# fabiocarrara/neural-ode-features

Measured on AMD Instinct MI355X. Metric: images/sec (fwd+adjoint) CIFAR-10 ODE-ResNet bs=128 at 1/2/4/8 GPU, higher is better.
Workload: dtype f32

## Files before the change

neural-ode-features_amd/csrc/kernels_head.hip:

```cpp
#include "node_internal.h"
#include "../../include/node_hip.h"
#include <cstdio>

namespace node {

namespace {
constexpr int HEAD_MAXIT = 16;

template <int CTRL>
__device__ inline float dpp_add(float v) {
  return v + __builtin_bit_cast(float, __builtin_amdgcn_update_dpp(0, __builtin_bit_cast(int, v), CTRL, 0xf, 0xf, true));
}
template <int LPC>
__device__ inline float lanes_sum(float v) {
  if (LPC >= 4) { v = dpp_add<0xB1>(v); v = dpp_add<0x4E>(v); }
  if (LPC >= 16) { v = dpp_add<0x141>(v); v = dpp_add<0x140>(v); }
  if (LPC >= 64) {
    v = v + __builtin_bit_cast(float, __builtin_amdgcn_update_dpp(0, __builtin_bit_cast(int, v), 0x142, 0xa, 0xf, false));
    v = v + __builtin_bit_cast(float, __builtin_amdgcn_update_dpp(0, __builtin_bit_cast(int, v), 0x143, 0xc, 0xf, false));
    v = __builtin_bit_cast(float, __builtin_amdgcn_readlane(__builtin_bit_cast(int, v), 63));
  }
  return v;
}

__device__ inline void groups_from_channels(const float* chv, float* grp, int G, int cpg) {
  __syncthreads();
  for (int g = threadIdx.x; g < G; g += blockDim.x) {
    float s = 0.f;
    for (int k = 0; k < cpg; ++k) s += chv[g * cpg + k];
    grp[g] = s;
  }
  __syncthreads();
}

__device__ inline float block_sum_256h(float v, float* red) {
  v = lanes_sum<64>(v);
  __syncthreads();
  if ((threadIdx.x & 63) == 0) red[threadIdx.x >> 6] = v;
  __syncthreads();
  return (red[0] + red[1]) + (red[2] + red[3]);
}

__device__ inline float group_sum(float v, float* ch, int c, int c_lo, int cpg, bool on) {
  __syncthreads();
  if (on) ch[c] = v;
  __syncthreads();
  float s = 0.f;
  if (on)
    for (int k = 0; k < cpg; ++k) s += ch[c_lo + k];
  return s;
}
}

template <int LPC>
__global__ __launch_bounds__(256) void k_head_fwd_v(const float* __restrict__ z, const float* __restrict__ gamma,
                                                    const float* __restrict__ beta, const float* __restrict__ scale,
                                                    float* __restrict__ pooled, float* __restrict__ stats, int C, int HW,
                                                    int G, float eps) {
  extern __shared__ float sm[];
  float* chv = sm;
  float* grp = sm + C;
  float* grp2 = grp + G;
  constexpr int CPP = 256 / LPC;
  const int n = blockIdx.x, cpg = C / G;
  const int lc = threadIdx.x / LPC, lq = threadIdx.x % LPC;
  const int q4 = HW >> 2;
  const int iters = (C + CPP - 1) / CPP;
  const float4* zs = reinterpret_cast<const float4*>(z + (size_t)n * C * HW);
  float4 v[HEAD_MAXIT];
#pragma unroll
  for (int i = 0; i < HEAD_MAXIT; ++i) {
    const int c = i * CPP + lc;
    v[i] = (i < iters && c < C) ? zs[(size_t)c * q4 + lq] : make_float4(0.f, 0.f, 0.f, 0.f);
  }
  const float inv_m = 1.0f / (float)(cpg * HW);
#pragma unroll
  for (int i = 0; i < HEAD_MAXIT; ++i) {
    const int c = i * CPP + lc;
    const float s = lanes_sum<LPC>((v[i].x + v[i].y) + (v[i].z + v[i].w));
    if (i < iters && c < C && lq == 0) chv[c] = s;
  }
  groups_from_channels(chv, grp, G, cpg);
#pragma unroll
  for (int i = 0; i < HEAD_MAXIT; ++i) {
    const int c = i * CPP + lc;
    const float mean = (i < iters && c < C) ? grp[c / cpg] * inv_m : 0.f;
    const float a = v[i].x - mean, b = v[i].y - mean, cc = v[i].z - mean, dd = v[i].w - mean;
    const float s = lanes_sum<LPC>((a * a + b * b) + (cc * cc + dd * dd));
    if (i < iters && c < C && lq == 0) chv[c] = s;
  }
  groups_from_channels(chv, grp2, G, cpg);
#pragma unroll
  for (int i = 0; i < HEAD_MAXIT; ++i) {
    const int c = i * CPP + lc;
    if (i < iters && c < C) {
      const int g = c / cpg;
      const float mean = grp[g] * inv_m, rstd = 1.0f / sqrtf(grp2[g] * inv_m + eps);
      const float gm = gamma[c], bt = beta[c];
      float acc = fmaxf(((v[i].x - mean) * rstd) * gm + bt, 0.f) + fmaxf(((v[i].y - mean) * rstd) * gm + bt, 0.f) +
                  fmaxf(((v[i].z - mean) * rstd) * gm + bt, 0.f) + fmaxf(((v[i].w - mean) * rstd) * gm + bt, 0.f);
      acc = lanes_sum<LPC>(acc) * (1.0f / (float)HW);
      if (lq == 0) {
        if (scale) acc *= scale[(size_t)n * C + c];
        pooled[(size_t)n * C + c] = acc;
        if (c == g * cpg) { stats[((size_t)n * G + g) * 2] = mean; stats[((size_t)n * G + g) * 2 + 1] = rstd; }
      }
    } else {
      (void)lanes_sum<LPC>(0.f);
    }
  }
}

template <int LPC>
__global__ __launch_bounds__(256) void k_head_bwd_v(const float* __restrict__ z, const float* __restrict__ gamma,
                                                    const float* __restrict__ beta, const float* __restrict__ scale,
                                                    const float* __restrict__ stats, const float* __restrict__ gpool,
                                                    float* __restrict__ dz, float* __restrict__ gpart, int C, int HW, int G) {
  extern __shared__ float sm[];
  float* chv = sm;
  float* chw = sm + C;
  float* grp = chw + C;
  float* grp2 = grp + G;
  constexpr int CPP = 256 / LPC;
  const int n = blockIdx.x, cpg = C / G;
  const int lc = threadIdx.x / LPC, lq = threadIdx.x % LPC;
  const int q4 = HW >> 2;
  const int iters = (C + CPP - 1) / CPP;
  const float4* zs = reinterpret_cast<const float4*>(z + (size_t)n * C * HW);
  float4* dzs = reinterpret_cast<float4*>(dz + (size_t)n * C * HW);
  const float inv_m = 1.0f / (float)(cpg * HW);
  float4 xh[HEAD_MAXIT];
  float gvv[HEAD_MAXIT];
#pragma unroll
  for (int i = 0; i < HEAD_MAXIT; ++i) {
    const int c = i * CPP + lc;
    const bool on = i < iters && c < C;
    float4 zv = on ? zs[(size_t)c * q4 + lq] : make_float4(0.f, 0.f, 0.f, 0.f);
    const int g = on ? c / cpg : 0;
    const float mean = on ? stats[((size_t)n * G + g) * 2] : 0.f, rstd = on ? stats[((size_t)n * G + g) * 2 + 1] : 0.f;
    xh[i] = make_float4((zv.x - mean) * rstd, (zv.y - mean) * rstd, (zv.z - mean) * rstd, (zv.w - mean) * rstd);
    float gv = 0.f;
    if (on) {
      gv = gpool[(size_t)n * C + c] * (1.0f / (float)HW);
      if (scale) gv *= scale[(size_t)n * C + c];
    }
    gvv[i] = gv;
    const float gm = on ? gamma[c] : 0.f, bt = on ? beta[c] : 0.f;
    const float g0 = (xh[i].x * gm + bt > 0.f) ? gv : 0.f, g1 = (xh[i].y * gm + bt > 0.f) ? gv : 0.f;
    const float g2 = (xh[i].z * gm + bt > 0.f) ? gv : 0.f, g3 = (xh[i].w * gm + bt > 0.f) ? gv : 0.f;
    const float dg = lanes_sum<LPC>((g0 * xh[i].x + g1 * xh[i].y) + (g2 * xh[i].z + g3 * xh[i].w));
    const float db = lanes_sum<LPC>((g0 + g1) + (g2 + g3));
    if (on && lq == 0) {
      gpart[((size_t)n * 2 + 0) * C + c] = dg;
      gpart[((size_t)n * 2 + 1) * C + c] = db;
      chv[c] = db * gm;
      chw[c] = dg * gm;
    }
  }
  __syncthreads();
  for (int g = threadIdx.x; g < G; g += 256) {
    float s1 = 0.f, s2 = 0.f;
    for (int k = 0; k < cpg; ++k) { s1 += chv[g * cpg + k]; s2 += chw[g * cpg + k]; }
    grp[g] = s1 * inv_m;
    grp2[g] = s2 * inv_m;
  }
  __syncthreads();
#pragma unroll
  for (int i = 0; i < HEAD_MAXIT; ++i) {
    const int c = i * CPP + lc;
    if (i < iters && c < C) {
      const int g = c / cpg;
      const float rstd = stats[((size_t)n * G + g) * 2 + 1], m1 = grp[g], m2 = grp2[g];
      const float gm = gamma[c], bt = beta[c], gv = gvv[i];
      float4 o;
      o.x = rstd * (((xh[i].x * gm + bt > 0.f) ? gv * gm : 0.f) - m1 - xh[i].x * m2);
      o.y = rstd * (((xh[i].y * gm + bt > 0.f) ? gv * gm : 0.f) - m1 - xh[i].y * m2);
      o.z = rstd * (((xh[i].z * gm + bt > 0.f) ? gv * gm : 0.f) - m1 - xh[i].z * m2);
      o.w = rstd * (((xh[i].w * gm + bt > 0.f) ? gv * gm : 0.f) - m1 - xh[i].w * m2);
      dzs[(size_t)c * q4 + lq] = o;
    }
  }
}

__global__ __launch_bounds__(256) void k_head_fwd_g(const float* __restrict__ z, const float* __restrict__ gamma,
                                                    const float* __restrict__ beta, const float* __restrict__ scale,
                                                    float* __restrict__ pooled, float* __restrict__ stats, int C, int HW,
                                                    int G, float eps) {
  extern __shared__ float ch[];
  const int n = blockIdx.x, cpg = C / G;
  const float inv_m = 1.0f / (float)(cpg * HW);
  for (int cb = 0; cb < C; cb += 256) {
    const int c = cb + threadIdx.x;
    const bool on = c < C;
    const int g = on ? c / cpg : 0, c_lo = g * cpg;
    const float* zc = z + ((size_t)n * C + (on ? c : 0)) * HW;
    float s = 0.f;
    if (on)
      for (int p = 0; p < HW; ++p) s += zc[p];
    const float mean = group_sum(s, ch, c, c_lo, cpg, on) * inv_m;
    float s2 = 0.f;
    if (on)
      for (int p = 0; p < HW; ++p) { const float dv = zc[p] - mean; s2 += dv * dv; }
    const float var = group_sum(s2, ch, c, c_lo, cpg, on) * inv_m;
    const float rstd = 1.0f / sqrtf(var + eps);
    if (on) {
      const float gm = gamma[c], bt = beta[c];
      float acc = 0.f;
      for (int p = 0; p < HW; ++p) acc += fmaxf(((zc[p] - mean) * rstd) * gm + bt, 0.f);
      acc *= 1.0f / (float)HW;
      if (scale) acc *= scale[(size_t)n * C + c];
      pooled[(size_t)n * C + c] = acc;
      if (c == c_lo) { stats[((size_t)n * G + g) * 2] = mean; stats[((size_t)n * G + g) * 2 + 1] = rstd; }
    }
  }
}

__global__ __launch_bounds__(256) void k_head_bwd_g(const float* __restrict__ z, const float* __restrict__ gamma,
                                                    const float* __restrict__ beta, const float* __restrict__ scale,
                                                    const float* __restrict__ stats, const float* __restrict__ gpool,
                                                    float* __restrict__ dz, float* __restrict__ gpart, int C, int HW, int G) {
  extern __shared__ float ch[];
  const int n = blockIdx.x, cpg = C / G;
  const float inv_m = 1.0f / (float)(cpg * HW);
  for (int cb = 0; cb < C; cb += 256) {
    const int c = cb + threadIdx.x;
    const bool on = c < C;
    const int g = on ? c / cpg : 0, c_lo = g * cpg;
    const size_t base = ((size_t)n * C + (on ? c : 0)) * HW;
    const float mean = on ? stats[((size_t)n * G + g) * 2] : 0.f, rstd = on ? stats[((size_t)n * G + g) * 2 + 1] : 0.f;
    const float gm = on ? gamma[c] : 0.f, bt = on ? beta[c] : 0.f;
    float gv = 0.f;
    if (on) {
      gv = gpool[(size_t)n * C + c] * (1.0f / (float)HW);
      if (scale) gv *= scale[(size_t)n * C + c];
    }
    float dg = 0.f, db = 0.f;
    if (on)
      for (int p = 0; p < HW; ++p) {
        const float xh = (z[base + p] - mean) * rstd;
        const float gu = (xh * gm + bt > 0.f) ? gv : 0.f;
        dg += gu * xh;
        db += gu;
      }
    if (on) {
      gpart[((size_t)n * 2 + 0) * C + c] = dg;
      gpart[((size_t)n * 2 + 1) * C + c] = db;
    }
    const float m1 = group_sum(db * gm, ch, c, c_lo, cpg, on) * inv_m;
    const float m2 = group_sum(dg * gm, ch, c, c_lo, cpg, on) * inv_m;
    if (on)
      for (int p = 0; p < HW; ++p) {
        const float xh = (z[base + p] - mean) * rstd;
        const float gu = (xh * gm + bt > 0.f) ? gv : 0.f;
        dz[base + p] = rstd * (gu * gm - m1 - xh * m2);
      }
  }
}

__global__ __launch_bounds__(256) void k_gn_relu_fwd(const float* __restrict__ z, const float* __restrict__ gamma,
                                                     const float* __restrict__ beta, float* __restrict__ out,
                                                     float* __restrict__ stats, int C, int HW, int G, float eps, int relu) {
  __shared__ float red[4];
  const int n = blockIdx.x / G, g = blockIdx.x - n * G, cpg = C / G;
  const int M = cpg * HW;
  const size_t base = ((size_t)n * C + (size_t)g * cpg) * HW;
  const float* zg = z + base;
  float s = 0.f;
  for (int i = threadIdx.x; i < M; i += 256) s += zg[i];
  const float mean = block_sum_256h(s, red) / (float)M;
  float s2 = 0.f;
  for (int i = threadIdx.x; i < M; i += 256) { const float dv = zg[i] - mean; s2 += dv * dv; }
  const float rstd = 1.0f / sqrtf(block_sum_256h(s2, red) / (float)M + eps);
  if (threadIdx.x == 0) { stats[(size_t)blockIdx.x * 2] = mean; stats[(size_t)blockIdx.x * 2 + 1] = rstd; }
  for (int cc = 0; cc < cpg; ++cc) {
    const float gm = gamma[g * cpg + cc], bt = beta[g * cpg + cc];
    for (int p = threadIdx.x; p < HW; p += 256) {
      float v = ((zg[cc * HW + p] - mean) * rstd) * gm + bt;
      if (relu) v = fmaxf(v, 0.f);
      out[base + cc * HW + p] = v;
    }
  }
}

__global__ __launch_bounds__(256) void k_gn_relu_bwd(const float* __restrict__ z, const float* __restrict__ gamma,
                                                     const float* __restrict__ beta, const float* __restrict__ stats,
                                                     const float* __restrict__ gout, float* __restrict__ dz,
                                                     float* __restrict__ gpart, int C, int HW, int G, int relu) {
  __shared__ float red[4];
  const int n = blockIdx.x / G, g = blockIdx.x - n * G, cpg = C / G;
  const int M = cpg * HW;
  const size_t base = ((size_t)n * C + (size_t)g * cpg) * HW;
  const float mean = stats[(size_t)blockIdx.x * 2], rstd = stats[(size_t)blockIdx.x * 2 + 1];
  float s1 = 0.f, s2 = 0.f;
  for (int cc = 0; cc < cpg; ++cc) {
    const int c = g * cpg + cc;
    const float gm = gamma[c], bt = beta[c];
    float dg = 0.f, db = 0.f;
    for (int p = threadIdx.x; p < HW; p += 256) {
      const float xh = (z[base + cc * HW + p] - mean) * rstd;
      float gu = gout[base + cc * HW + p];
      if (relu && !(xh * gm + bt > 0.f)) gu = 0.f;
      dg += gu * xh;
      db += gu;
    }
    dg = block_sum_256h(dg, red);
    db = block_sum_256h(db, red);
    if (threadIdx.x == 0) {
      gpart[((size_t)n * 2 + 0) * C + c] = dg;
      gpart[((size_t)n * 2 + 1) * C + c] = db;
    }
    s1 += db * gm;
    s2 += dg * gm;
  }
  const float m1 = s1 / (float)M, m2 = s2 / (float)M;
  for (int cc = 0; cc < cpg; ++cc) {
    const float gm = gamma[g * cpg + cc], bt = beta[g * cpg + cc];
    for (int p = threadIdx.x; p < HW; p += 256) {
      const float xh = (z[base + cc * HW + p] - mean) * rstd;
      float gu = gout[base + cc * HW + p];
      if (relu && !(xh * gm + bt > 0.f)) gu = 0.f;
      dz[base + cc * HW + p] = rstd * (gu * gm - m1 - xh * m2);
    }
  }
}

void launch_gn_relu_fwd(const node_shape& sh, const float* z, const float* gamma, const float* beta, int relu, float* out,
                        float* stats, hipStream_t s) {
  hipLaunchKernelGGL(k_gn_relu_fwd, dim3(sh.n * sh.groups), dim3(256), 0, s, z, gamma, beta, out, stats, sh.c, sh.h * sh.w,
                     sh.groups, sh.eps, relu);
}
void launch_gn_relu_bwd(const node_shape& sh, const float* z, const float* gamma, const float* beta, const float* stats,
                        int relu, const float* gout, float* dz, float* gpart, hipStream_t s) {
  hipLaunchKernelGGL(k_gn_relu_bwd, dim3(sh.n * sh.groups), dim3(256), 0, s, z, gamma, beta, stats, gout, dz, gpart, sh.c,
                     sh.h * sh.w, sh.groups, relu);
}

int head_check(const node_shape* sh, char* why, size_t why_len) {
  if (!sh) { snprintf(why, why_len, "shape is NULL"); return NODE_ERR_NULL; }
  if (sh->n <= 0 || sh->c <= 0 || sh->h <= 0 || sh->w <= 0 || sh->groups <= 0) { snprintf(why, why_len, "non-positive dimension"); return NODE_ERR_SHAPE; }
  if (sh->c % sh->groups != 0) { snprintf(why, why_len, "groups (%d) must divide channels (%d)", sh->groups, sh->c); return NODE_ERR_SHAPE; }
  const int cpg = sh->c / sh->groups;
  if (sh->c > 256 && 256 % cpg != 0) { snprintf(why, why_len, "C = %d with %d channels per group: groups would straddle the 256-channel passes", sh->c, cpg); return NODE_ERR_UNSUPPORTED; }
  if ((size_t)sh->c * sizeof(float) > 24 * 1024) { snprintf(why, why_len, "C = %d does not fit the LDS scratch", sh->c); return NODE_ERR_UNSUPPORTED; }
  return NODE_OK;
}

static int head_lpc(const node_shape& sh) {
  const int HW = sh.h * sh.w;
  if (HW % 4 != 0) return 0;
  const int q4 = HW / 4;
  if (q4 != 1 && q4 != 4 && q4 != 16 && q4 != 64) return 0;
  const int cpp = 256 / q4;
  if ((sh.c + cpp - 1) / cpp > HEAD_MAXIT) return 0;
  return q4;
}

void launch_head_fwd(const node_shape& sh, const float* z, const float* gamma, const float* beta, const float* scale,
                     float* pooled, float* stats, hipStream_t s) {
  const int HW = sh.h * sh.w;
  const size_t lds = (size_t)(sh.c + 2 * sh.groups) * sizeof(float);
#define HEAD_FWD(LPC) hipLaunchKernelGGL((k_head_fwd_v<LPC>), dim3(sh.n), dim3(256), lds, s, z, gamma, beta, scale, pooled, stats, sh.c, HW, sh.groups, sh.eps)
  switch (head_lpc(sh)) {
    case 1: HEAD_FWD(1); return;
    case 4: HEAD_FWD(4); return;
    case 16: HEAD_FWD(16); return;
    case 64: HEAD_FWD(64); return;
    default: break;
  }
#undef HEAD_FWD
  hipLaunchKernelGGL(k_head_fwd_g, dim3(sh.n), dim3(256), (size_t)sh.c * sizeof(float), s, z, gamma, beta, scale, pooled, stats,
                     sh.c, HW, sh.groups, sh.eps);
}
__global__ __launch_bounds__(256) void k_head_gsum(const float* __restrict__ gpart, float* __restrict__ gsum, int N, int W) {
  __shared__ float red[4][64];
  const int col = blockIdx.x * 64 + (threadIdx.x & 63), part = threadIdx.x >> 6;
  float s = 0.f;
  if (col < W)
    for (int n = part; n < N; n += 4) s += gpart[(size_t)n * W + col];
  red[part][threadIdx.x & 63] = s;
  __syncthreads();
  if (part == 0 && col < W) gsum[col] = (red[0][threadIdx.x] + red[1][threadIdx.x]) + (red[2][threadIdx.x] + red[3][threadIdx.x]);
}
void launch_head_gsum(const float* gpart, float* gsum, int N, int C, hipStream_t s) {
  hipLaunchKernelGGL(k_head_gsum, dim3((2 * C + 63) / 64), dim3(256), 0, s, gpart, gsum, N, 2 * C);
}

void launch_head_bwd(const node_shape& sh, const float* z, const float* gamma, const float* beta, const float* scale,
                     const float* stats, const float* gpool, float* dz, float* gpart, hipStream_t s) {
  const int HW = sh.h * sh.w;
  const size_t lds = (size_t)(2 * sh.c + 2 * sh.groups) * sizeof(float);
#define HEAD_BWD(LPC) hipLaunchKernelGGL((k_head_bwd_v<LPC>), dim3(sh.n), dim3(256), lds, s, z, gamma, beta, scale, stats, gpool, dz, gpart, sh.c, HW, sh.groups)
  switch (head_lpc(sh)) {
    case 1: HEAD_BWD(1); return;
    case 4: HEAD_BWD(4); return;
    case 16: HEAD_BWD(16); return;
    case 64: HEAD_BWD(64); return;
    default: break;
  }
#undef HEAD_BWD
  hipLaunchKernelGGL(k_head_bwd_g, dim3(sh.n), dim3(256), (size_t)sh.c * sizeof(float), s, z, gamma, beta, scale, stats, gpool, dz,
                     gpart, sh.c, HW, sh.groups);
}

}
```

neural-ode-features_amd/csrc/kernels_optim.hip:

```cpp
#include "node_internal.h"

namespace node {

__global__ __launch_bounds__(256) void k_sgd_multi(SgdTable tb, float lr, float momentum, float wd, float gscale, const float* skip) {
  if (skip != nullptr && *skip != 0.f) return;
  const SgdEntry e = tb.e[blockIdx.y];
  float* __restrict__ p = e.p;
  const float* __restrict__ g = e.g;
  float* __restrict__ m = e.m;
  const size_t n = e.n;
  const size_t stride = (size_t)gridDim.x * 256;
  const size_t start = (size_t)blockIdx.x * 256 + threadIdx.x;
  const bool vec = (((uintptr_t)p | (uintptr_t)g | (uintptr_t)m) & 15) == 0;
  size_t done = 0;
  if (m == nullptr) {
    for (size_t i = start; i < n; i += stride) p[i] -= lr * (gscale * g[i] + wd * p[i]);
    return;
  }
  if (vec) {
    const size_t n4 = n >> 2;
    float4* p4 = reinterpret_cast<float4*>(p);
    const float4* g4 = reinterpret_cast<const float4*>(g);
    float4* m4 = reinterpret_cast<float4*>(m);
    for (size_t i = start; i < n4; i += stride) {
      float4 pv = p4[i];
      const float4 gv = g4[i];
      float4 mv = m4[i];
      mv.x = momentum * mv.x + (gscale * gv.x + wd * pv.x);
      mv.y = momentum * mv.y + (gscale * gv.y + wd * pv.y);
      mv.z = momentum * mv.z + (gscale * gv.z + wd * pv.z);
      mv.w = momentum * mv.w + (gscale * gv.w + wd * pv.w);
      pv.x -= lr * mv.x; pv.y -= lr * mv.y; pv.z -= lr * mv.z; pv.w -= lr * mv.w;
      p4[i] = pv;
      m4[i] = mv;
    }
    done = n4 << 2;
  }
  for (size_t i = done + start; i < n; i += stride) {
    const float b = momentum * m[i] + (gscale * g[i] + wd * p[i]);
    m[i] = b;
    p[i] -= lr * b;
  }
}

void launch_sgd_multi(const SgdTable& tb, int count, size_t max_n, float lr, float momentum, float wd, float gscale,
                      const float* skip, hipStream_t s) {
  size_t bx = (max_n / 4 + 255) / 256;
  if (bx > 64) bx = 64;
  if (bx < 1) bx = 1;
  hipLaunchKernelGGL(k_sgd_multi, dim3((unsigned)bx, (unsigned)count), dim3(256), 0, s, tb, lr, momentum, wd, gscale, skip);
}


__device__ inline double pow_whole(double b, float t) {
  double r = 1.0;
  for (unsigned k = (unsigned)t; k != 0; k >>= 1) {
    if (k & 1) r *= b;
    b *= b;
  }
  return r;
}

struct AdamCoef { float gscale, wd, w1, b2, w2, step_size, sqrt_c2, eps; };

__device__ inline void adam_elem(float& p, float g, float& m, float& v, const AdamCoef& c) {
  g = c.gscale * g + c.wd * p;
  m = m + c.w1 * (g - m);
  v = c.b2 * v + (c.w2 * g) * g;
  p = p - c.step_size * (m / (sqrtf(v) / c.sqrt_c2 + c.eps));
}

__global__ __launch_bounds__(256) void k_adam_multi(AdamTable tb, float lr, double b1, double b2, float eps, float wd, float gscale,
                                                    const float* skip) {
  if (skip != nullptr && *skip != 0.f) return;
  const AdamEntry e = tb.e[blockIdx.y];
  float* __restrict__ p = e.p;
  const float* __restrict__ g = e.g;
  float* __restrict__ m = e.m;
  float* __restrict__ v = e.v;
  const size_t n = e.n;
  const size_t stride = (size_t)gridDim.x * 256;
  const size_t start = (size_t)blockIdx.x * 256 + threadIdx.x;
  const float t = *e.step + 1.f;
  const double c1 = 1.0 - pow_whole(b1, t), c2 = 1.0 - pow_whole(b2, t);
  const AdamCoef c = {gscale, wd, (float)(1.0 - b1), (float)b2, (float)(1.0 - b2), (float)((double)lr / c1), (float)sqrt(c2), eps};
  const bool vec = (((uintptr_t)p | (uintptr_t)g | (uintptr_t)m | (uintptr_t)v) & 15) == 0;
  size_t done = 0;
  if (vec) {
    const size_t n4 = n >> 2;
    float4* p4 = reinterpret_cast<float4*>(p);
    const float4* g4 = reinterpret_cast<const float4*>(g);
    float4* m4 = reinterpret_cast<float4*>(m);
    float4* v4 = reinterpret_cast<float4*>(v);
    for (size_t i = start; i < n4; i += stride) {
      float4 pv = p4[i];
      const float4 gv = g4[i];
      float4 mv = m4[i];
      float4 vv = v4[i];
      adam_elem(pv.x, gv.x, mv.x, vv.x, c);
      adam_elem(pv.y, gv.y, mv.y, vv.y, c);
      adam_elem(pv.z, gv.z, mv.z, vv.z, c);
      adam_elem(pv.w, gv.w, mv.w, vv.w, c);
      p4[i] = pv;
      m4[i] = mv;
      v4[i] = vv;
    }
    done = n4 << 2;
  }
  for (size_t i = done + start; i < n; i += stride) {
    float pv = p[i], mv = m[i], vv = v[i];
    adam_elem(pv, g[i], mv, vv, c);
    p[i] = pv;
    m[i] = mv;
    v[i] = vv;
  }
}

__global__ __launch_bounds__(ADAM_TABLE) void k_adam_advance(AdamTable tb, int count, const float* skip) {
  if (skip != nullptr && *skip != 0.f) return;
  if ((int)threadIdx.x < count) *tb.e[threadIdx.x].step += 1.f;
}

void launch_adam_multi(const AdamTable& tb, int count, size_t max_n, float lr, double b1, double b2, float eps, float wd,
                       float gscale, const float* skip, hipStream_t s) {
  size_t bx = (max_n / 4 + 255) / 256;
  if (bx > 64) bx = 64;
  if (bx < 1) bx = 1;
  hipLaunchKernelGGL(k_adam_multi, dim3((unsigned)bx, (unsigned)count), dim3(256), 0, s, tb, lr, b1, b2, eps, wd, gscale, skip);
  hipLaunchKernelGGL(k_adam_advance, dim3(1), dim3(ADAM_TABLE), 0, s, tb, count, skip);
}

}
```

neural-ode-features_amd/csrc/kernels_theta_finalize.hip:

```cpp
#include "theta_finalize.h"

namespace node {

__global__ __launch_bounds__(256) void k_theta_finalize(ThetaFinalizeArgs a, Dims d) {
  if (a.ctrl->done) return;
  theta_finalize_body<256>(a, d, blockIdx.x, gridDim.x);
}

void launch_theta_finalize(const Dims& d, const ThetaFinalizeArgs& a, hipStream_t s) {
  hipLaunchKernelGGL(k_theta_finalize, dim3(theta_finalize_blocks(d, a)), dim3(256), 0, s, a, d);
}

}
```

neural-ode-features_amd/csrc/theta_finalize.h:

```cpp
#pragma once
#include "pointwise_common.h"
#include "wino4.h"

namespace node {

template <typename T>
__device__ __forceinline__ T tf_sel2(const T (&x)[2], int i) { return i ? x[1] : x[0]; }
template <typename T>
__device__ __forceinline__ T tf_sel3(const T (&x)[3], int i) { return i == 0 ? x[0] : i == 1 ? x[1] : x[2]; }

template <int BT>
__device__ __forceinline__ void theta_finalize_body(const ThetaFinalizeArgs& a, const Dims& d, const int bx_all, const int nblk) {
  static_assert(BT == 256 || BT == 128, "a row group is one wave: four of them in one or two per thread");
  __shared__ float red[256];
  __shared__ int s_last;
  const int tid = threadIdx.x;
  const ThetaLayout L = theta_layout(d.C);
  const int C = d.C;
  const int nsm = (9 * C + 63) / 64;
  const int wb = (nblk - 5 * nsm) / 2;
  if (bx_all >= 5 * nsm) {
    const int layer = (bx_all - 5 * nsm) / wb, bx = (bx_all - 5 * nsm) - layer * wb;
    const size_t CC = (size_t)C * C;
    const size_t n4 = 9 * CC / 4;
    const float4* wp = reinterpret_cast<const float4*>(tf_sel2(a.wpart, layer));
    float4* out = reinterpret_cast<float4*>(a.theta_out + tf_sel2(L.wc, layer));
    const size_t stride = (size_t)wb * 256;
    if (a.dU != nullptr) {
      const size_t cc4 = CC / 4;
      const float4* du = reinterpret_cast<const float4*>(a.dU + (size_t)layer * W4_COMPS * CC);
      for (int h = 0; h < 256; h += BT)
      for (size_t i = (size_t)bx * 256 + h + tid; i < cc4; i += stride) {
        const unsigned off = (unsigned)i * 16u;
        float4 tq[6][3];
#pragma unroll
        for (int xi = 0; xi < 6; ++xi) {
          float4 u[6];
#pragma unroll
          for (int nu = 0; nu < 6; ++nu) u[nu] = *reinterpret_cast<const float4*>(reinterpret_cast<const char*>(du + (size_t)(xi * 6 + nu) * cc4) + off);
#pragma unroll
          for (int kw = 0; kw < 3; ++kw) {
            float4 s = make_float4(0.f, 0.f, 0.f, 0.f);
#pragma unroll
            for (int nu = 0; nu < 6; ++nu) {
              const float gq = (float)W4_G[nu][kw];
              if (gq != 0.f) { s.x += gq * u[nu].x; s.y += gq * u[nu].y; s.z += gq * u[nu].z; s.w += gq * u[nu].w; }
            }
            tq[xi][kw] = s;
          }
        }
#pragma unroll
        for (int kh = 0; kh < 3; ++kh)
#pragma unroll
          for (int kw = 0; kw < 3; ++kw) {
            float4 s = make_float4(0.f, 0.f, 0.f, 0.f);
#pragma unroll
            for (int xi = 0; xi < 6; ++xi) {
              const float gq = (float)W4_G[xi][kh];
              if (gq != 0.f) { s.x += gq * tq[xi][kw].x; s.y += gq * tq[xi][kw].y; s.z += gq * tq[xi][kw].z; s.w += gq * tq[xi][kw].w; }
            }
            *reinterpret_cast<float4*>(reinterpret_cast<char*>(out + (size_t)(kh * 3 + kw) * cc4) + off) = make_float4(a.osign * s.x, a.osign * s.y, a.osign * s.z, a.osign * s.w);
          }
      }
      return;
    }
    for (int h = 0; h < 256; h += BT)
    for (size_t i = (size_t)bx * 256 + h + tid; i < n4; i += stride) {
      float4 acc = make_float4(0.f, 0.f, 0.f, 0.f);
      int sp = 0;
      for (; sp + 4 <= d.nsplit; sp += 4) {
        const float4 v0 = wp[(size_t)sp * n4 + i], v1 = wp[(size_t)(sp + 1) * n4 + i];
        const float4 v2 = wp[(size_t)(sp + 2) * n4 + i], v3 = wp[(size_t)(sp + 3) * n4 + i];
        acc.x += (v0.x + v1.x) + (v2.x + v3.x); acc.y += (v0.y + v1.y) + (v2.y + v3.y);
        acc.z += (v0.z + v1.z) + (v2.z + v3.z); acc.w += (v0.w + v1.w) + (v2.w + v3.w);
      }
      for (; sp < d.nsplit; ++sp) {
        const float4 v = wp[(size_t)sp * n4 + i];
        acc.x += v.x; acc.y += v.y; acc.z += v.z; acc.w += v.w;
      }
      out[i] = make_float4(a.osign * acc.x, a.osign * acc.y, a.osign * acc.z, a.osign * acc.w);
    }
    return;
  }
  const int job = bx_all / nsm, bxs = bx_all - job * nsm;
  const bool gn = job < 3;
  const int layer = gn ? job : job - 3;
  const int ncol = gn ? 2 * C : 9 * C;
  if (bxs * 64 >= ncol) return;
  const int rows = gn ? tf_sel3(a.gpart_rows, layer) : (a.spart_rows > 0 ? a.spart_rows : d.N);
  const float* src = gn ? tf_sel3(a.gpart, layer) : tf_sel2(a.spart, layer);
  const int cl = tid & 63, rg = tid >> 6;
  const int col = bxs * 64 + cl;
  float vr[256 / BT];
#pragma unroll
  for (int g = 0; g < 256 / BT; ++g) {
    float v = 0.f;
    if (col < ncol) {
      int r = rg + g * (BT / 64);
      for (; r + 12 < rows; r += 16) {
        const float v0 = src[(size_t)r * ncol + col], v1 = src[(size_t)(r + 4) * ncol + col];
        const float v2 = src[(size_t)(r + 8) * ncol + col], v3 = src[(size_t)(r + 12) * ncol + col];
        v += (v0 + v1) + (v2 + v3);
      }
      for (; r < rows; r += 4) v += src[(size_t)r * ncol + col];
    }
    vr[g] = v;
  }
#pragma unroll
  for (int g = 0; g < 256 / BT; ++g) red[g * BT + tid] = vr[g];
  __syncthreads();
  if (rg != 0) return;
  const bool on = col < ncol;
  const float v = (red[cl] + red[64 + cl]) + (red[128 + cl] + red[192 + cl]);
  if (gn) {
    if (on) {
      const int which = col >= C ? 1 : 0;
      a.theta_out[(which ? tf_sel3(L.b, layer) : tf_sel3(L.g, layer)) + (col - which * C)] = a.osign * v;
    }
    return;
  }
  if (on) {
    a.theta_out[tf_sel2(L.wt, layer) + col] = a.osign * (v * eval_time(a.et));
    if (col >= 4 * C && col < 5 * C) a.theta_out[tf_sel2(L.cb, layer) + (col - 4 * C)] = a.osign * v;
  }
  const int nb = (9 * C + 63) / 64;
  float* dotpart = a.sred + (size_t)2 * 9 * C;
  unsigned* counter = reinterpret_cast<unsigned*>(dotpart + 2 * nb);
  const float part = wave_sum(on ? v * tf_sel2(a.wtime, layer)[col] : 0.f);
#if defined(__HIP_DEVICE_COMPILE__) && !defined(__gfx950__)
#error "k_theta_finalize's fence-free hand-off is only valid on gfx950: use release/acquire on the counter elsewhere"
#endif
  if (cl == 0) {
    __hip_atomic_store(dotpart + layer * nb + bxs, part, __ATOMIC_RELAXED, __HIP_MEMORY_SCOPE_AGENT);
    asm volatile("s_waitcnt vmcnt(0)" ::: "memory");
    s_last = __hip_atomic_fetch_add(counter, 1u, __ATOMIC_RELAXED, __HIP_MEMORY_SCOPE_AGENT) == (unsigned)(2 * nb - 1);
  }
  __builtin_amdgcn_wave_barrier();
  if (!s_last) return;
  float tot = 0.f;
  for (int i = cl; i < 2 * nb; i += 64) tot += __hip_atomic_load(dotpart + i, __ATOMIC_RELAXED, __HIP_MEMORY_SCOPE_AGENT);
  tot = wave_sum(tot);
  if (cl == 0) {
    __hip_atomic_store(counter, 0u, __ATOMIC_RELAXED, __HIP_MEMORY_SCOPE_AGENT);
    if (a.write_scalar) a.ctrl->ts_k[a.kidx] = a.osign * tot;
    if (a.vjp_t_out) *a.vjp_t_out = a.osign * tot;
  }
}

inline unsigned theta_finalize_blocks(const Dims& d, const ThetaFinalizeArgs& a) {
  size_t wblocks = (9 * (size_t)d.C * d.C / 4 + 255) / 256;
  if (a.dU != nullptr) wblocks = ((size_t)d.C * d.C / 4 + 255) / 256;
  if (wblocks > 1024) wblocks = 1024;
  const size_t nsmall = (9 * (size_t)d.C + 63) / 64;
  return (unsigned)(5 * nsmall + 2 * wblocks);
}

}
```

Baseline: 29750.

## Split head GroupNorm across group blocks, chunk SGD jobs, batch column-sum loads

The head forward and backward kernels now launch several blocks per sample, each owning a contiguous range of GroupNorm groups, so the grid reaches about 512 blocks instead of one per sample. The SGD kernel is changed to a flat job list with fixed-size chunks per tensor, found by binary search, replacing the 2D grid with a per-tensor stride loop. The gsum and theta-finalize column reductions now issue 32 loads ahead before accumulating, to expose more memory-level parallelism. Summation order changes slightly, and register pressure in the batched-load loops rises.

```diff
diff --git a/neural-ode-features_amd/csrc/kernels_head.hip b/neural-ode-features_amd/csrc/kernels_head.hip
--- a/neural-ode-features_amd/csrc/kernels_head.hip
+++ b/neural-ode-features_amd/csrc/kernels_head.hip
@@ -23,9 +23,9 @@
   return v;
 }
 
-__device__ inline void groups_from_channels(const float* chv, float* grp, int G, int cpg) {
-  __syncthreads();
-  for (int g = threadIdx.x; g < G; g += blockDim.x) {
+__device__ inline void groups_from_channels(const float* chv, float* grp, int g0, int G, int cpg) {
+  __syncthreads();
+  for (int g = g0 + threadIdx.x; g < G; g += blockDim.x) {
     float s = 0.f;
     for (int k = 0; k < cpg; ++k) s += chv[g * cpg + k];
     grp[g] = s;
@@ -56,44 +56,46 @@
 __global__ __launch_bounds__(256) void k_head_fwd_v(const float* __restrict__ z, const float* __restrict__ gamma,
                                                     const float* __restrict__ beta, const float* __restrict__ scale,
                                                     float* __restrict__ pooled, float* __restrict__ stats, int C, int HW,
-                                                    int G, float eps) {
+                                                    int G, float eps, int S, int gpw) {
   extern __shared__ float sm[];
   float* chv = sm;
   float* grp = sm + C;
   float* grp2 = grp + G;
   constexpr int CPP = 256 / LPC;
-  const int n = blockIdx.x, cpg = C / G;
+  const int n = blockIdx.x / S, part = blockIdx.x - n * S, cpg = C / G;
+  const int g0 = part * gpw, g1 = g0 + gpw < G ? g0 + gpw : G;
+  const int c0 = g0 * cpg, c1 = g1 * cpg;
   const int lc = threadIdx.x / LPC, lq = threadIdx.x % LPC;
   const int q4 = HW >> 2;
-  const int iters = (C + CPP - 1) / CPP;
+  const int iters = (c1 - c0 + CPP - 1) / CPP;
   const float4* zs = reinterpret_cast<const float4*>(z + (size_t)n * C * HW);
   float4 v[HEAD_MAXIT];
 #pragma unroll
   for (int i = 0; i < HEAD_MAXIT; ++i) {
-    const int c = i * CPP + lc;
-    v[i] = (i < iters && c < C) ? zs[(size_t)c * q4 + lq] : make_float4(0.f, 0.f, 0.f, 0.f);
+    const int c = c0 + i * CPP + lc;
+    v[i] = (i < iters && c < c1) ? zs[(size_t)c * q4 + lq] : make_float4(0.f, 0.f, 0.f, 0.f);
   }
   const float inv_m = 1.0f / (float)(cpg * HW);
 #pragma unroll
   for (int i = 0; i < HEAD_MAXIT; ++i) {
-    const int c = i * CPP + lc;
+    const int c = c0 + i * CPP + lc;
     const float s = lanes_sum<LPC>((v[i].x + v[i].y) + (v[i].z + v[i].w));
-    if (i < iters && c < C && lq == 0) chv[c] = s;
-  }
-  groups_from_channels(chv, grp, G, cpg);
-#pragma unroll
-  for (int i = 0; i < HEAD_MAXIT; ++i) {
-    const int c = i * CPP + lc;
-    const float mean = (i < iters && c < C) ? grp[c / cpg] * inv_m : 0.f;
+    if (i < iters && c < c1 && lq == 0) chv[c] = s;
+  }
+  groups_from_channels(chv, grp, g0, g1, cpg);
+#pragma unroll
+  for (int i = 0; i < HEAD_MAXIT; ++i) {
+    const int c = c0 + i * CPP + lc;
+    const float mean = (i < iters && c < c1) ? grp[c / cpg] * inv_m : 0.f;
     const float a = v[i].x - mean, b = v[i].y - mean, cc = v[i].z - mean, dd = v[i].w - mean;
     const float s = lanes_sum<LPC>((a * a + b * b) + (cc * cc + dd * dd));
-    if (i < iters && c < C && lq == 0) chv[c] = s;
-  }
-  groups_from_channels(chv, grp2, G, cpg);
-#pragma unroll
-  for (int i = 0; i < HEAD_MAXIT; ++i) {
-    const int c = i * CPP + lc;
-    if (i < iters && c < C) {
+    if (i < iters && c < c1 && lq == 0) chv[c] = s;
+  }
+  groups_from_channels(chv, grp2, g0, g1, cpg);
+#pragma unroll
+  for (int i = 0; i < HEAD_MAXIT; ++i) {
+    const int c = c0 + i * CPP + lc;
+    if (i < iters && c < c1) {
       const int g = c / cpg;
       const float mean = grp[g] * inv_m, rstd = 1.0f / sqrtf(grp2[g] * inv_m + eps);
       const float gm = gamma[c], bt = beta[c];
@@ -115,17 +117,20 @@
 __global__ __launch_bounds__(256) void k_head_bwd_v(const float* __restrict__ z, const float* __restrict__ gamma,
                                                     const float* __restrict__ beta, const float* __restrict__ scale,
                                                     const float* __restrict__ stats, const float* __restrict__ gpool,
-                                                    float* __restrict__ dz, float* __restrict__ gpart, int C, int HW, int G) {
+                                                    float* __restrict__ dz, float* __restrict__ gpart, int C, int HW, int G,
+                                                    int S, int gpw) {
   extern __shared__ float sm[];
   float* chv = sm;
   float* chw = sm + C;
   float* grp = chw + C;
   float* grp2 = grp + G;
   constexpr int CPP = 256 / LPC;
-  const int n = blockIdx.x, cpg = C / G;
+  const int n = blockIdx.x / S, part = blockIdx.x - n * S, cpg = C / G;
+  const int g0 = part * gpw, g1 = g0 + gpw < G ? g0 + gpw : G;
+  const int c0 = g0 * cpg, c1 = g1 * cpg;
   const int lc = threadIdx.x / LPC, lq = threadIdx.x % LPC;
   const int q4 = HW >> 2;
-  const int iters = (C + CPP - 1) / CPP;
+  const int iters = (c1 - c0 + CPP - 1) / CPP;
   const float4* zs = reinterpret_cast<const float4*>(z + (size_t)n * C * HW);
   float4* dzs = reinterpret_cast<float4*>(dz + (size_t)n * C * HW);
   const float inv_m = 1.0f / (float)(cpg * HW);
@@ -133,8 +138,8 @@
   float gvv[HEAD_MAXIT];
 #pragma unroll
   for (int i = 0; i < HEAD_MAXIT; ++i) {
-    const int c = i * CPP + lc;
-    const bool on = i < iters && c < C;
+    const int c = c0 + i * CPP + lc;
+    const bool on = i < iters && c < c1;
     float4 zv = on ? zs[(size_t)c * q4 + lq] : make_float4(0.f, 0.f, 0.f, 0.f);
     const int g = on ? c / cpg : 0;
     const float mean = on ? stats[((size_t)n * G + g) * 2] : 0.f, rstd = on ? stats[((size_t)n * G + g) * 2 + 1] : 0.f;
@@ -158,7 +163,7 @@
     }
   }
   __syncthreads();
-  for (int g = threadIdx.x; g < G; g += 256) {
+  for (int g = g0 + threadIdx.x; g < g1; g += 256) {
     float s1 = 0.f, s2 = 0.f;
     for (int k = 0; k < cpg; ++k) { s1 += chv[g * cpg + k]; s2 += chw[g * cpg + k]; }
     grp[g] = s1 * inv_m;
@@ -167,8 +172,8 @@
   __syncthreads();
 #pragma unroll
   for (int i = 0; i < HEAD_MAXIT; ++i) {
-    const int c = i * CPP + lc;
-    if (i < iters && c < C) {
+    const int c = c0 + i * CPP + lc;
+    if (i < iters && c < c1) {
       const int g = c / cpg;
       const float rstd = stats[((size_t)n * G + g) * 2 + 1], m1 = grp[g], m2 = grp2[g];
       const float gm = gamma[c], bt = beta[c], gv = gvv[i];
@@ -355,11 +360,20 @@
   return q4;
 }
 
+static void head_split(const node_shape& sh, int& S, int& gpw) {
+  int want = (512 + sh.n - 1) / sh.n;
+  if (want > sh.groups) want = sh.groups;
+  gpw = (sh.groups + want - 1) / want;
+  S = (sh.groups + gpw - 1) / gpw;
+}
+
 void launch_head_fwd(const node_shape& sh, const float* z, const float* gamma, const float* beta, const float* scale,
                      float* pooled, float* stats, hipStream_t s) {
   const int HW = sh.h * sh.w;
   const size_t lds = (size_t)(sh.c + 2 * sh.groups) * sizeof(float);
-#define HEAD_FWD(LPC) hipLaunchKernelGGL((k_head_fwd_v<LPC>), dim3(sh.n), dim3(256), lds, s, z, gamma, beta, scale, pooled, stats, sh.c, HW, sh.groups, sh.eps)
+  int S, gpw;
+  head_split(sh, S, gpw);
+#define HEAD_FWD(LPC) hipLaunchKernelGGL((k_head_fwd_v<LPC>), dim3(sh.n * S), dim3(256), lds, s, z, gamma, beta, scale, pooled, stats, sh.c, HW, sh.groups, sh.eps, S, gpw)
   switch (head_lpc(sh)) {
     case 1: HEAD_FWD(1); return;
     case 4: HEAD_FWD(4); return;
@@ -371,12 +385,20 @@
   hipLaunchKernelGGL(k_head_fwd_g, dim3(sh.n), dim3(256), (size_t)sh.c * sizeof(float), s, z, gamma, beta, scale, pooled, stats,
                      sh.c, HW, sh.groups, sh.eps);
 }
+constexpr int GSUM_BLK = 32;
 __global__ __launch_bounds__(256) void k_head_gsum(const float* __restrict__ gpart, float* __restrict__ gsum, int N, int W) {
   __shared__ float red[4][64];
   const int col = blockIdx.x * 64 + (threadIdx.x & 63), part = threadIdx.x >> 6;
   float s = 0.f;
   if (col < W)
-    for (int n = part; n < N; n += 4) s += gpart[(size_t)n * W + col];
+    for (int nb = part; nb < N; nb += 4 * GSUM_BLK) {
+      float t[GSUM_BLK];
+#pragma unroll
+      for (int k = 0; k < GSUM_BLK; ++k) t[k] = nb + 4 * k < N ? gpart[(size_t)(nb + 4 * k) * W + col] : 0.f;
+#pragma unroll
+      for (int k = 0; k < GSUM_BLK; ++k)
+        if (nb + 4 * k < N) s += t[k];
+    }
   red[part][threadIdx.x & 63] = s;
   __syncthreads();
   if (part == 0 && col < W) gsum[col] = (red[0][threadIdx.x] + red[1][threadIdx.x]) + (red[2][threadIdx.x] + red[3][threadIdx.x]);
@@ -389,7 +411,9 @@
                      const float* stats, const float* gpool, float* dz, float* gpart, hipStream_t s) {
   const int HW = sh.h * sh.w;
   const size_t lds = (size_t)(2 * sh.c + 2 * sh.groups) * sizeof(float);
-#define HEAD_BWD(LPC) hipLaunchKernelGGL((k_head_bwd_v<LPC>), dim3(sh.n), dim3(256), lds, s, z, gamma, beta, scale, stats, gpool, dz, gpart, sh.c, HW, sh.groups)
+  int S, gpw;
+  head_split(sh, S, gpw);
+#define HEAD_BWD(LPC) hipLaunchKernelGGL((k_head_bwd_v<LPC>), dim3(sh.n * S), dim3(256), lds, s, z, gamma, beta, scale, stats, gpool, dz, gpart, sh.c, HW, sh.groups, S, gpw)
   switch (head_lpc(sh)) {
     case 1: HEAD_BWD(1); return;
     case 4: HEAD_BWD(4); return;
diff --git a/neural-ode-features_amd/csrc/kernels_optim.hip b/neural-ode-features_amd/csrc/kernels_optim.hip
--- a/neural-ode-features_amd/csrc/kernels_optim.hip
+++ b/neural-ode-features_amd/csrc/kernels_optim.hip
@@ -2,53 +2,109 @@
 
 namespace node {
 
-__global__ __launch_bounds__(256) void k_sgd_multi(SgdTable tb, float lr, float momentum, float wd, float gscale, const float* skip) {
+constexpr int OPT_U = 4;
+constexpr int OPT_CHUNK = 256 * OPT_U * 4;
+struct OptJobs { unsigned first[SGD_TABLE + 1]; };
+static_assert(ADAM_TABLE == SGD_TABLE, "one job table type for both optimizers");
+
+__device__ inline int opt_job_tensor(const OptJobs& jb, int count, unsigned bx) {
+  int lo = 0, hi = count - 1;
+  while (lo < hi) {
+    const int mid = (lo + hi + 1) >> 1;
+    if (jb.first[mid] <= bx) lo = mid; else hi = mid - 1;
+  }
+  return lo;
+}
+
+static unsigned opt_jobs(OptJobs& jb, int count, const size_t* n) {
+  unsigned total = 0;
+  for (int i = 0; i < count; ++i) {
+    jb.first[i] = total;
+    const size_t c = (n[i] + OPT_CHUNK - 1) / OPT_CHUNK;
+    total += c > 0 ? (unsigned)c : 1u;
+  }
+  for (int i = count; i <= SGD_TABLE; ++i) jb.first[i] = total;
+  return total;
+}
+
+template <typename T, typename F>
+__device__ __forceinline__ void sgd_chunk(T* __restrict__ p, const T* __restrict__ g, T* __restrict__ m, size_t lo, size_t hi, F&& step) {
+  T pv[OPT_U], gv[OPT_U], mv[OPT_U];
+#pragma unroll
+  for (int u = 0; u < OPT_U; ++u) {
+    const size_t i = lo + u * 256 + threadIdx.x;
+    if (i < hi) { pv[u] = p[i]; gv[u] = g[i]; mv[u] = m[i]; }
+  }
+#pragma unroll
+  for (int u = 0; u < OPT_U; ++u) {
+    const size_t i = lo + u * 256 + threadIdx.x;
+    if (i < hi) {
+      step(pv[u], gv[u], mv[u]);
+      p[i] = pv[u];
+      m[i] = mv[u];
+    }
+  }
+}
+
+__global__ __launch_bounds__(256) void k_sgd_multi(SgdTable tb, OptJobs jb, int count, float lr, float momentum, float wd, float gscale,
+                                                   const float* skip) {
   if (skip != nullptr && *skip != 0.f) return;
-  const SgdEntry e = tb.e[blockIdx.y];
+  const int t = opt_job_tensor(jb, count, blockIdx.x);
+  const SgdEntry e = tb.e[t];
   float* __restrict__ p = e.p;
   const float* __restrict__ g = e.g;
   float* __restrict__ m = e.m;
   const size_t n = e.n;
-  const size_t stride = (size_t)gridDim.x * 256;
-  const size_t start = (size_t)blockIdx.x * 256 + threadIdx.x;
-  const bool vec = (((uintptr_t)p | (uintptr_t)g | (uintptr_t)m) & 15) == 0;
-  size_t done = 0;
+  const size_t chunk = blockIdx.x - jb.first[t];
   if (m == nullptr) {
-    for (size_t i = start; i < n; i += stride) p[i] -= lr * (gscale * g[i] + wd * p[i]);
+    const size_t lo = chunk * OPT_CHUNK, hi = lo + OPT_CHUNK < n ? lo + OPT_CHUNK : n;
+    for (size_t b = lo; b < hi; b += 256 * OPT_U) {
+      float pv[OPT_U], gv[OPT_U];
+#pragma unroll
+      for (int u = 0; u < OPT_U; ++u) {
+        const size_t i = b + u * 256 + threadIdx.x;
+        if (i < hi) { pv[u] = p[i]; gv[u] = g[i]; }
+      }
+#pragma unroll
+      for (int u = 0; u < OPT_U; ++u) {
+        const size_t i = b + u * 256 + threadIdx.x;
+        if (i < hi) p[i] = pv[u] - lr * (gscale * gv[u] + wd * pv[u]);
+      }
+    }
     return;
   }
+  auto step1 = [&](float& pv, const float& gv, float& mv) {
+    mv = momentum * mv + (gscale * gv + wd * pv);
+    pv -= lr * mv;
+  };
+  const bool vec = (((uintptr_t)p | (uintptr_t)g | (uintptr_t)m) & 15) == 0;
   if (vec) {
     const size_t n4 = n >> 2;
-    float4* p4 = reinterpret_cast<float4*>(p);
-    const float4* g4 = reinterpret_cast<const float4*>(g);
-    float4* m4 = reinterpret_cast<float4*>(m);
-    for (size_t i = start; i < n4; i += stride) {
-      float4 pv = p4[i];
-      const float4 gv = g4[i];
-      float4 mv = m4[i];
-      mv.x = momentum * mv.x + (gscale * gv.x + wd * pv.x);
-      mv.y = momentum * mv.y + (gscale * gv.y + wd * pv.y);
-      mv.z = momentum * mv.z + (gscale * gv.z + wd * pv.z);
-      mv.w = momentum * mv.w + (gscale * gv.w + wd * pv.w);
-      pv.x -= lr * mv.x; pv.y -= lr * mv.y; pv.z -= lr * mv.z; pv.w -= lr * mv.w;
-      p4[i] = pv;
-      m4[i] = mv;
+    const size_t lo = chunk * (OPT_CHUNK / 4), hi = lo + OPT_CHUNK / 4 < n4 ? lo + OPT_CHUNK / 4 : n4;
+    sgd_chunk(reinterpret_cast<float4*>(p), reinterpret_cast<const float4*>(g), reinterpret_cast<float4*>(m), lo, hi,
+              [&](float4& pv, const float4& gv, float4& mv) {
+                step1(pv.x, gv.x, mv.x); step1(pv.y, gv.y, mv.y); step1(pv.z, gv.z, mv.z); step1(pv.w, gv.w, mv.w);
+              });
+    if (chunk == 0 && (n4 << 2) + threadIdx.x < n) {
+      const size_t i = (n4 << 2) + threadIdx.x;
+      const float b = momentum * m[i] + (gscale * g[i] + wd * p[i]);
+      m[i] = b;
+      p[i] -= lr * b;
     }
-    done = n4 << 2;
+    return;
   }
-  for (size_t i = done + start; i < n; i += stride) {
-    const float b = momentum * m[i] + (gscale * g[i] + wd * p[i]);
-    m[i] = b;
-    p[i] -= lr * b;
-  }
+  const size_t lo = chunk * OPT_CHUNK, hi = lo + OPT_CHUNK < n ? lo + OPT_CHUNK : n;
+  for (size_t b = lo; b < hi; b += 256 * OPT_U) sgd_chunk(p, g, m, b, hi, step1);
 }
 
 void launch_sgd_multi(const SgdTable& tb, int count, size_t max_n, float lr, float momentum, float wd, float gscale,
                       const float* skip, hipStream_t s) {
-  size_t bx = (max_n / 4 + 255) / 256;
-  if (bx > 64) bx = 64;
-  if (bx < 1) bx = 1;
-  hipLaunchKernelGGL(k_sgd_multi, dim3((unsigned)bx, (unsigned)count), dim3(256), 0, s, tb, lr, momentum, wd, gscale, skip);
+  (void)max_n;
+  OptJobs jb;
+  size_t n[SGD_TABLE];
+  for (int i = 0; i < count; ++i) n[i] = tb.e[i].n;
+  const unsigned jobs = opt_jobs(jb, count, n);
+  hipLaunchKernelGGL(k_sgd_multi, dim3(jobs), dim3(256), 0, s, tb, jb, count, lr, momentum, wd, gscale, skip);
 }
 
 
diff --git a/neural-ode-features_amd/csrc/kernels_theta_finalize.hip b/neural-ode-features_amd/csrc/kernels_theta_finalize.hip
--- a/neural-ode-features_amd/csrc/kernels_theta_finalize.hip
+++ b/neural-ode-features_amd/csrc/kernels_theta_finalize.hip
@@ -4,7 +4,7 @@
 
 __global__ __launch_bounds__(256) void k_theta_finalize(ThetaFinalizeArgs a, Dims d) {
   if (a.ctrl->done) return;
-  theta_finalize_body<256>(a, d, blockIdx.x, gridDim.x);
+  theta_finalize_body<256, true>(a, d, blockIdx.x, gridDim.x);
 }
 
 void launch_theta_finalize(const Dims& d, const ThetaFinalizeArgs& a, hipStream_t s) {
diff --git a/neural-ode-features_amd/csrc/theta_finalize.h b/neural-ode-features_amd/csrc/theta_finalize.h
--- a/neural-ode-features_amd/csrc/theta_finalize.h
+++ b/neural-ode-features_amd/csrc/theta_finalize.h
@@ -9,7 +9,7 @@
 template <typename T>
 __device__ __forceinline__ T tf_sel3(const T (&x)[3], int i) { return i == 0 ? x[0] : i == 1 ? x[1] : x[2]; }
 
-template <int BT>
+template <int BT, bool AHEAD = false>
 __device__ __forceinline__ void theta_finalize_body(const ThetaFinalizeArgs& a, const Dims& d, const int bx_all, const int nblk) {
   static_assert(BT == 256 || BT == 128, "a row group is one wave: four of them in one or two per thread");
   __shared__ float red[256];
@@ -92,19 +92,48 @@
   const int cl = tid & 63, rg = tid >> 6;
   const int col = bxs * 64 + cl;
   float vr[256 / BT];
-#pragma unroll
-  for (int g = 0; g < 256 / BT; ++g) {
+  if constexpr (AHEAD) {
+    static_assert(BT == 256, "one row group per thread");
+    constexpr int TF_BLK = 32;
     float v = 0.f;
     if (col < ncol) {
-      int r = rg + g * (BT / 64);
-      for (; r + 12 < rows; r += 16) {
-        const float v0 = src[(size_t)r * ncol + col], v1 = src[(size_t)(r + 4) * ncol + col];
-        const float v2 = src[(size_t)(r + 8) * ncol + col], v3 = src[(size_t)(r + 12) * ncol + col];
-        v += (v0 + v1) + (v2 + v3);
+      const unsigned off = (unsigned)(rg * ncol + col) * 4u, step = (unsigned)ncol * 16u;
+      for (int rb = 0; rb < rows; rb += 4 * TF_BLK) {
+        const char* base = reinterpret_cast<const char*>(src + (size_t)rb * ncol);
+        const int r0 = rb + rg;
+        float t[TF_BLK];
+#pragma unroll
+        for (int k = 0; k < TF_BLK; ++k)
+          t[k] = r0 + 4 * k < rows ? *reinterpret_cast<const float*>(base + (off + (unsigned)k * step)) : 0.f;
+#pragma unroll
+        for (int q = 0; q < TF_BLK / 4; ++q) {
+          const int r = r0 + 16 * q;
+          if (r + 12 < rows) {
+            v += (t[4 * q] + t[4 * q + 1]) + (t[4 * q + 2] + t[4 * q + 3]);
+          } else {
+#pragma unroll
+            for (int k = 0; k < 4; ++k)
+              if (r + 4 * k < rows) v += t[4 * q + k];
+          }
+        }
       }
-      for (; r < rows; r += 4) v += src[(size_t)r * ncol + col];
     }
-    vr[g] = v;
+    vr[0] = v;
+  } else {
+#pragma unroll
+    for (int g = 0; g < 256 / BT; ++g) {
+      float v = 0.f;
+      if (col < ncol) {
+        int r = rg + g * (BT / 64);
+        for (; r + 12 < rows; r += 16) {
+          const float v0 = src[(size_t)r * ncol + col], v1 = src[(size_t)(r + 4) * ncol + col];
+          const float v2 = src[(size_t)(r + 8) * ncol + col], v3 = src[(size_t)(r + 12) * ncol + col];
+          v += (v0 + v1) + (v2 + v3);
+        }
+        for (; r < rows; r += 4) v += src[(size_t)r * ncol + col];
+      }
+      vr[g] = v;
+    }
   }
 #pragma unroll
   for (int g = 0; g < 256 / BT; ++g) red[g * BT + tid] = vr[g];
```

After: 29920 (median of 6 runs). About the same (+0.6%).
